# wangjunchi/LLMSeg

Measured on AMD Instinct MI355X. Metric: images/sec (1024x1024, 64-tok prompt) model_forward fwd+bwd, higher is better.
Workload: dtype bf16; 1 GPU; BASELINE.json configs[2]: synthetic 1024x1024 + random-init LLaVA-7B(Llama-7B+CLIP-L/14)/SAM-ViT-H, batch_size=2 per GPU, fwd+bwd train step (CE + align + IoP losses, LoRA r=8 dropout 0.05 on q/v + trainable embed/lm_head/text_fcs/lisa_*, frozen towers, fp32 gradient arena, AdamW step every 10 micro-steps inside the timed region, micro-step replayed from a hipGraph), 256 candidate masks, 64-token ; global_batch=2, parallelism=dp1, graph=True, valid=True

## Files before the change

llmseg_amd/csrc/backward.hip:

```cpp
#include <algorithm>
#include <cstdlib>
#include "common.h"
#include "llmseg_hip.h"

namespace {

inline unsigned grid_for(long total) {
  long g = (total + 255) / 256;
  return (unsigned)(g < 1 ? 1 : (g > 8192 ? 8192 : g));
}

__global__ __launch_bounds__(256) void colsum_kernel(const bf16_t* __restrict__ x, float* __restrict__ out, float* __restrict__ part, long M, long N, long ld) {
  __shared__ float red[4][64];
  const int c = threadIdx.x & 63, rl = threadIdx.x >> 6;
  const long col = (long)blockIdx.x * 64 + c;
  const long rows_per = (M + gridDim.y - 1) / gridDim.y;
  const long r0 = (long)blockIdx.y * rows_per, r1 = min(M, r0 + rows_per);
  float s = 0.f;
  if (col < N)
    for (long r = r0 + rl; r < r1; r += 4) s += bf2f(x[r * ld + col]);
  red[rl][c] = s;
  __syncthreads();
  if (rl == 0 && col < N) {
    const float v = (red[0][c] + red[1][c]) + (red[2][c] + red[3][c]);
// ... 505 lines not shown
}

extern "C" int llmseg_ce_bwd(const void* logits, const int64_t* labels, const float* coef, void* dlogits, int32_t N, int32_t T, int64_t V, int64_t ldl,
                             void* stream) {
  LL_CHECK(logits && labels && coef && dlogits && N > 0 && T > 1 && V > 0 && ldl >= V, "ce_bwd: bad arguments");
  LL_LAUNCH_KERNEL(ce_bwd_kernel, dim3((unsigned)(N * T)), dim3(256), 0, (hipStream_t)stream, (const bf16_t*)logits, labels, coef, (bf16_t*)dlogits, T,
                     (long)V, (long)ldl);
  LL_LAUNCH_CHECK("ce_bwd");
  return LLMSEG_OK;
}

extern "C" int llmseg_scatter_add_rows(const void* src, const int64_t* idx, float* dst, int64_t n, int64_t cols, void* stream) {
  LL_CHECK(src && idx && dst && n > 0 && cols > 0, "scatter_add_rows: bad arguments");
  LL_CHECK(n < (1L << 31), "scatter_add_rows: too many source rows");
  LL_LAUNCH_KERNEL(scatter_add_rows_kernel, dim3((unsigned)n), dim3(256), 0, (hipStream_t)stream, (const bf16_t*)src, idx, dst, (long)n, (long)cols);
  LL_LAUNCH_CHECK("scatter_add_rows");
  return LLMSEG_OK;
}

extern "C" int llmseg_sumsq(const void* x, int64_t n, int is_f32, float* out, void* workspace, int64_t workspace_bytes, void* stream) {
  LL_CHECK(x && out && n > 0, "sumsq: bad arguments");
  LL_CHECK(workspace && workspace_bytes >= 4, "sumsq: workspace (>= 4 bytes, 8 KiB for every partial) is required");
  long g = std::min<long>(2048, (n + 2047) / 2048);
  g = std::max<long>(1, std::min<long>(g, workspace_bytes / 4));
  LL_LAUNCH_KERNEL(sumsq_kernel, dim3((unsigned)g), dim3(256), 0, (hipStream_t)stream, x, (long)n, is_f32, (float*)workspace);
  LL_LAUNCH_KERNEL(fold_column_kernel, dim3(1), dim3(256), 0, (hipStream_t)stream, (const float*)workspace, (long)g, out, 1.f);
  LL_LAUNCH_CHECK("sumsq");
  return LLMSEG_OK;
}

extern "C" int llmseg_adamw(void* p, float* master, const void* grad, int grad_f32, float* m, float* v, int64_t n, float lr, float beta1, float beta2,
                            float eps, float weight_decay, int64_t step, const float* grad_scale, void* stream) {
  LL_CHECK(p && master && grad && m && v && n > 0 && step > 0, "adamw: bad arguments");
  const float bc1 = 1.f - powf(beta1, (float)step), bc2 = 1.f - powf(beta2, (float)step);
  LL_LAUNCH_KERNEL(adamw_kernel, dim3(grid_for(n)), dim3(256), 0, (hipStream_t)stream, (bf16_t*)p, master, grad, grad_f32, m, v, (long)n, lr, beta1, beta2,
                     eps, weight_decay, bc1, bc2, grad_scale);
  LL_LAUNCH_CHECK("adamw");
  return LLMSEG_OK;
}

namespace {
constexpr int LR = 8;

struct DropP { const unsigned long* rng; uint32_t stream, thr; float scale; uint32_t seg; };

__device__ __forceinline__ unsigned long drop_index(const DropP& dp, unsigned long m, unsigned long width, unsigned long k, uint32_t& off_add) {
  off_add = 0;
  if (dp.seg) {
    off_add = (uint32_t)(m / dp.seg);
    m -= (unsigned long)off_add * dp.seg;
  }
  return (m * width + k) >> 3;
}

template <int RW>
__global__ __launch_bounds__(256) void lora_down_kernel(const bf16_t* __restrict__ x0, const bf16_t* __restrict__ x1, long ldx, const bf16_t* __restrict__ w0,
                                                       const bf16_t* __restrict__ w1, bf16_t* __restrict__ y, long ldy, long M, int K, int w_kr, float alpha,
                                                       int zero_cols, int nb, DropP dp) {
  const int lane = threadIdx.x & 63;
  const long m0 = ((long)blockIdx.x * 4 + (threadIdx.x >> 6)) * RW;
  if (m0 >= M) return;
  float acc[2][RW][LR];
#pragma unroll
  for (int b = 0; b < 2; ++b)
#pragma unroll
    for (int i = 0; i < RW; ++i)
#pragma unroll
      for (int r = 0; r < LR; ++r) acc[b][i][r] = 0.f;
  const bool same = x0 == x1;
#pragma unroll 2
  for (int k = lane * 8; k < K; k += 64 * 8) {
#pragma unroll
    for (int b = 0; b < 2; ++b) {
      if (b >= nb) break;
      const bf16_t* xb = b == 0 ? x0 : x1;
      const bf16_t* wb = b == 0 ? w0 : w1;
      float xv[RW][8], wv[8];
#pragma unroll
      for (int i = 0; i < RW; ++i) {
        const long m = min(m0 + i, M - 1);
        unpack8(*reinterpret_cast<const uint4*>(xb + m * ldx + k), xv[i]);
        if (dp.thr) {
          uint32_t oa;
          const unsigned long di = drop_index(dp, (unsigned long)m, (unsigned long)K, (unsigned long)k, oa);
          dropout8(xv[i], di, dp.stream + b, dp.rng, dp.thr, dp.scale, oa);
        }
      }
      (void)same;
      if (w_kr) {
#pragma unroll
        for (int j = 0; j < 8; ++j) {
          unpack8(*reinterpret_cast<const uint4*>(wb + (long)(k + j) * LR), wv);
#pragma unroll
          for (int i = 0; i < RW; ++i)
#pragma unroll
            for (int r = 0; r < LR; ++r) acc[b][i][r] += xv[i][j] * wv[r];
        }
      } else {
#pragma unroll
        for (int r = 0; r < LR; ++r) {
          unpack8(*reinterpret_cast<const uint4*>(wb + (long)r * K + k), wv);
#pragma unroll
          for (int i = 0; i < RW; ++i)
#pragma unroll
            for (int j = 0; j < 8; ++j) acc[b][i][r] += xv[i][j] * wv[j];
        }
      }
    }
  }
#pragma unroll
  for (int i = 0; i < RW; ++i) {
#pragma unroll
    for (int b = 0; b < 2; ++b)
#pragma unroll
      for (int r = 0; r < LR; ++r) acc[b][i][r] = wave_sum(acc[b][i][r]) * alpha;
    if (m0 + i < M) {
      bf16_t* yr = y + (m0 + i) * ldy;
      if (lane == 0) *reinterpret_cast<uint4*>(yr) = pack8(acc[0][i]);
      else if (lane == 1 && nb > 1) *reinterpret_cast<uint4*>(yr + 8) = pack8(acc[1][i]);
      else if (lane >= nb && (lane - nb) * 8 < zero_cols) *reinterpret_cast<uint4*>(yr + lane * 8) = make_uint4(0, 0, 0, 0);
    }
  }
}

__global__ __launch_bounds__(256) void lora_down_mfma_kernel(const bf16_t* __restrict__ x0, const bf16_t* __restrict__ x1, long ldx, const bf16_t* __restrict__ w0,
                                                            const bf16_t* __restrict__ w1, bf16_t* __restrict__ y, long ldy, long M, int K, float alpha,
                                                            int zero_cols, int nb, DropP dp, float* __restrict__ part) {
  __shared__ float red[4][2][8][16];
  __shared__ float fin[16][16];
  const int lane = threadIdx.x & 63, wave = threadIdx.x >> 6;
  const int r = lane & 15, kc = lane >> 4;
  const long m0 = (long)blockIdx.x * 16;
  const long m = min(m0 + r, M - 1);
  const int kq = K / (4 * (int)gridDim.y);
  const int kbeg = ((int)blockIdx.y * 4 + wave) * kq;
  const bool same = x0 == x1;
  f32x4_t acc0 = {0.f, 0.f, 0.f, 0.f}, acc1 = {0.f, 0.f, 0.f, 0.f};
  auto masked = [&](uint4 v, unsigned long idx, uint32_t stream, uint32_t off_add) {
    const unsigned long seed = dp.rng[0], off = dp.rng[1] + off_add;
    const Philox8 ph = philox4x32_10((uint32_t)idx, (uint32_t)(idx >> 32), stream, (uint32_t)off, (uint32_t)seed, (uint32_t)(seed >> 32));
    uint32_t* u = reinterpret_cast<uint32_t*>(&v);
#pragma unroll
    for (int j = 0; j < 4; ++j) {
      const uint32_t lo = (ph.w[j] & 0xffffu) >= dp.thr ? 0x0000ffffu : 0u, hi = (ph.w[j] >> 16) >= dp.thr ? 0xffff0000u : 0u;
      u[j] &= lo | hi;
    }
    return v;
  };
#pragma unroll 4
  for (int k = kbeg + kc * 8; k < kbeg + kq; k += 32) {
    uint4 xa = *reinterpret_cast<const uint4*>(x0 + m * ldx + k);
    uint4 xb = (nb > 1 && !same) ? *reinterpret_cast<const uint4*>(x1 + m * ldx + k) : xa;
    const uint4 wa = r < LR ? *reinterpret_cast<const uint4*>(w0 + (long)r * K + k) : make_uint4(0, 0, 0, 0);
    const uint4 wb = (nb > 1 && r < LR) ? *reinterpret_cast<const uint4*>(w1 + (long)r * K + k) : make_uint4(0, 0, 0, 0);
    if (dp.thr) {
      uint32_t oa;
      const unsigned long idx = drop_index(dp, (unsigned long)m, (unsigned long)K, (unsigned long)k, oa);
      xa = masked(xa, idx, dp.stream, oa);
      if (nb > 1) xb = masked(xb, idx, dp.stream + 1, oa);
    }
    acc0 = __builtin_amdgcn_mfma_f32_16x16x32_bf16(__builtin_bit_cast(bf16x8_t, wa), __builtin_bit_cast(bf16x8_t, xa), acc0, 0, 0, 0);
    if (nb > 1) acc1 = __builtin_amdgcn_mfma_f32_16x16x32_bf16(__builtin_bit_cast(bf16x8_t, wb), __builtin_bit_cast(bf16x8_t, xb), acc1, 0, 0, 0);
  }
  if (kc < 2) {
#pragma unroll
    for (int e = 0; e < 4; ++e) { red[wave][0][4 * kc + e][r] = acc0[e]; red[wave][1][4 * kc + e][r] = acc1[e]; }
  }
  __syncthreads();
  {
    const int b = threadIdx.x >> 7, rank = (threadIdx.x >> 4) & 7, mm = threadIdx.x & 15;
    const float sum = (red[0][b][rank][mm] + red[1][b][rank][mm]) + (red[2][b][rank][mm] + red[3][b][rank][mm]);
    if (part) {
      if (m0 + mm < M) part[((long)blockIdx.y * M + m0 + mm) * 16 + b * 8 + rank] = sum;
    } else fin[mm][b * 8 + rank] = sum * alpha * (dp.thr ? dp.scale : 1.f);
  }
  if (part) return;
  __syncthreads();
  const int nch = nb + zero_cols / 8;
  for (int t = threadIdx.x; t < 16 * nch; t += blockDim.x) {
    const int mm = t / nch, ch = t - mm * nch;
    if (m0 + mm >= M) continue;
    uint4 o = make_uint4(0, 0, 0, 0);
    if (ch < nb) o = pack8(&fin[mm][ch * 8]);
    *reinterpret_cast<uint4*>(y + (m0 + mm) * ldy + ch * 8) = o;
  }
}

__device__ __forceinline__ void lora_down_finish_body(const float* __restrict__ part, int S, bf16_t* __restrict__ y, long ldy, long M, float scale,
                                                      int zero_cols, int nb, long bid, long nblocks) {
  const int nch = nb + zero_cols / 8;
  const long total = M * nch;
  for (long t = bid * blockDim.x + threadIdx.x; t < total; t += nblocks * blockDim.x) {
    const long mm = t / nch;
    const int ch = (int)(t - mm * nch);
    uint4 o = make_uint4(0, 0, 0, 0);
    if (ch < nb) {
      float v[8];
#pragma unroll
      for (int e = 0; e < 8; ++e) v[e] = 0.f;
      for (int s2 = 0; s2 < S; ++s2) {
        const float* pp = part + ((long)s2 * M + mm) * 16 + ch * 8;
#pragma unroll
        for (int e = 0; e < 8; ++e) v[e] += pp[e];
      }
#pragma unroll
      for (int e = 0; e < 8; ++e) v[e] *= scale;
      o = pack8(v);
    }
    *reinterpret_cast<uint4*>(y + mm * ldy + ch * 8) = o;
  }
}
__global__ __launch_bounds__(256) void lora_down_finish_kernel(const float* __restrict__ part, int S, bf16_t* __restrict__ y, long ldy, long M, float scale,
                                                              int zero_cols, int nb) {
  lora_down_finish_body(part, S, y, ldy, M, scale, zero_cols, nb, blockIdx.x, gridDim.x);
}

struct OuterP { const bf16_t* a[4]; const bf16_t* b[4]; float* out[4]; long lda[4], ldb[4]; int out_rn[4]; float alpha[4]; uint32_t drop[4]; };
__global__ __launch_bounds__(256) void lora_outer_kernel(OuterP q, long M, long N, DropP dp, float* __restrict__ part) {
  __shared__ float red[4][8][8 * LR];
  const int z = blockIdx.z;
  const bf16_t* __restrict__ a = q.a[z];
  const bf16_t* __restrict__ b = q.b[z];
  float* __restrict__ out = q.out[z];
  const long lda = q.lda[z], ldb = q.ldb[z];
  const int out_rn = q.out_rn[z];
  const float alpha = q.alpha[z];
  if (q.drop[z] == 0) dp.thr = 0;
  const uint32_t dstream = q.drop[z] - 1;
  const int lane = threadIdx.x & 63, wave = threadIdx.x >> 6;
  const int cl = lane & 7, rl = lane >> 3;
  const long n = ((long)blockIdx.x * 8 + cl) * 8;
  const long per = (M + gridDim.y * 4 - 1) / (gridDim.y * 4);
  const long m0 = ((long)blockIdx.y * 4 + wave) * per, m1 = min(M, m0 + per);
  const bool on = n < N;
  float acc[8][LR];
#pragma unroll
  for (int j = 0; j < 8; ++j)
#pragma unroll
    for (int r = 0; r < LR; ++r) acc[j][r] = 0.f;
  if (on) {
    long m = m0 + rl;
    for (; m + 16 < m1; m += 24) {
      uint4 av[3], bv[3];
#pragma unroll
      for (int u = 0; u < 3; ++u) {
        av[u] = *reinterpret_cast<const uint4*>(a + (m + 8 * u) * lda + n);
        bv[u] = *reinterpret_cast<const uint4*>(b + (m + 8 * u) * ldb);
      }
#pragma unroll
      for (int u = 0; u < 3; ++u) {
        float x[8], y[8];
        unpack8(av[u], x); unpack8(bv[u], y);
        if (dp.thr) {
          uint32_t oa;
          const unsigned long di = drop_index(dp, (unsigned long)(m + 8 * u), (unsigned long)N, (unsigned long)n, oa);
          dropout8(x, di, dstream, dp.rng, dp.thr, dp.scale, oa);
        }
#pragma unroll
        for (int j = 0; j < 8; ++j)
#pragma unroll
          for (int r = 0; r < LR; ++r) acc[j][r] = fmaf(x[j], y[r], acc[j][r]);
      }
    }
    for (; m < m1; m += 8) {
      float x[8], y[8];
      unpack8(*reinterpret_cast<const uint4*>(a + m * lda + n), x);
      unpack8(*reinterpret_cast<const uint4*>(b + m * ldb), y);
      if (dp.thr) {
        uint32_t oa;
        const unsigned long di = drop_index(dp, (unsigned long)m, (unsigned long)N, (unsigned long)n, oa);
        dropout8(x, di, dstream, dp.rng, dp.thr, dp.scale, oa);
      }
#pragma unroll
      for (int j = 0; j < 8; ++j)
#pragma unroll
        for (int r = 0; r < LR; ++r) acc[j][r] = fmaf(x[j], y[r], acc[j][r]);
    }
  }
#pragma unroll
  for (int j = 0; j < 8; ++j)
#pragma unroll
    for (int r = 0; r < LR; ++r) {
      float v = acc[j][r];
      v += __shfl_xor(v, 8, 64); v += __shfl_xor(v, 16, 64); v += __shfl_xor(v, 32, 64);
      acc[j][r] = v * alpha;
    }
  if (rl == 0) {
#pragma unroll
    for (int j = 0; j < 8; ++j)
#pragma unroll
      for (int r = 0; r < LR; ++r) red[wave][cl][j * LR + r] = acc[j][r];
  }
  __syncthreads();
  float* __restrict__ dstp = part ? part + ((long)blockIdx.y * gridDim.z + z) * N * LR : out;
  for (int idx = threadIdx.x; idx < 8 * 8 * LR; idx += blockDim.x) {
    const int c = idx / (8 * LR), jr = idx % (8 * LR), j = jr / LR, r = jr % LR;
    const long nn = ((long)blockIdx.x * 8 + c) * 8 + j;
    if (nn < N) {
      const float v = (red[0][c][jr] + red[1][c][jr]) + (red[2][c][jr] + red[3][c][jr]);
      const long cell = out_rn ? (long)r * N + nn : nn * LR + r;
      if (part) dstp[cell] = v;
      else dstp[cell] += v;
    }
  }
}

__global__ __launch_bounds__(256) void lora_apply_kernel(bf16_t* __restrict__ y, long ldy, const bf16_t* __restrict__ xa, long ldxa,
                                                        const bf16_t* __restrict__ w0, const bf16_t* __restrict__ w1, long M, long N, int w_rn,
                                                        float alpha, int nb, DropP dp) {
  const long nch = N >> 3, total = M * nch;
  for (long i = (long)blockIdx.x * blockDim.x + threadIdx.x; i < total; i += (long)gridDim.x * blockDim.x) {
    const long m = i / nch, c = i % nch;
    float yv[8], wv[8];
    unpack8(*reinterpret_cast<const uint4*>(y + m * ldy + c * 8), yv);
    for (int b = 0; b < nb; ++b) {
      const bf16_t* w = b == 0 ? w0 : w1;
      float xv[8], dv[8];
      unpack8(*reinterpret_cast<const uint4*>(xa + m * ldxa + 8 * b), xv);
      if (w_rn) {
#pragma unroll
        for (int j = 0; j < 8; ++j) dv[j] = 0.f;
#pragma unroll
        for (int r = 0; r < LR; ++r) {
          unpack8(*reinterpret_cast<const uint4*>(w + (long)r * N + c * 8), wv);
#pragma unroll
          for (int j = 0; j < 8; ++j) dv[j] += xv[r] * wv[j];
        }
      } else {
#pragma unroll
        for (int j = 0; j < 8; ++j) {
          unpack8(*reinterpret_cast<const uint4*>(w + (c * 8 + j) * LR), wv);
          float s = 0.f;
#pragma unroll
          for (int r = 0; r < LR; ++r) s += xv[r] * wv[r];
          dv[j] = s;
        }
      }
      if (dp.thr) {
        uint32_t oa;
        const unsigned long di = drop_index(dp, (unsigned long)m, (unsigned long)N, (unsigned long)(c * 8), oa);
        dropout8(dv, di, dp.stream + b, dp.rng, dp.thr, dp.scale, oa);
      }
#pragma unroll
      for (int j = 0; j < 8; ++j) yv[j] += alpha * dv[j];
    }
    *reinterpret_cast<uint4*>(y + m * ldy + c * 8) = pack8(yv);
  }
}

template <int CPT, bool LORA>
__global__ __launch_bounds__(256) void reduce_lora_normbwd_kernel(const float* __restrict__ slab, int S, long slab_sz, const bf16_t* __restrict__ x,
                                                                 const bf16_t* __restrict__ w, bf16_t* __restrict__ dx, long rows, int cols, float eps, int rms,
                                                                 const bf16_t* __restrict__ dres, bf16_t* __restrict__ xa, long ldxa,
                                                                 const bf16_t* __restrict__ w0, const bf16_t* __restrict__ w1, float alpha, int nb, DropP dp,
                                                                 const float* __restrict__ lp, int lS, float lscale, int lzero) {
  __shared__ float red[16];
  __shared__ float tl[16];
  const long row = blockIdx.x;
  const int nch = cols >> 3;
  const long N = cols;
  if (LORA && lp != nullptr) {
    if (threadIdx.x < 16) {
      float v = 0.f;
      if ((int)threadIdx.x < 8 * nb) {
        for (int s2 = 0; s2 < lS; ++s2) v += lp[((long)s2 * rows + row) * 16 + threadIdx.x];
        v *= lscale;
      }
      const bf16_t vb = f2bf(v);
      tl[threadIdx.x] = bf2f(vb);
      xa[row * ldxa + threadIdx.x] = vb;
    } else if ((int)threadIdx.x < 16 + lzero) xa[row * ldxa + threadIdx.x] = 0;
    __syncthreads();
  }
  uint4 xc[CPT], gc[CPT], wc[CPT];
#pragma unroll
  for (int i = 0; i < CPT; ++i) {
    const int c = threadIdx.x + 256 * i;
    xc[i] = gc[i] = wc[i] = make_uint4(0, 0, 0, 0);
    if (c < nch) {
      xc[i] = *reinterpret_cast<const uint4*>(x + row * cols + c * 8);
      wc[i] = *reinterpret_cast<const uint4*>(w + c * 8);
      const float* sp = slab + row * N + c * 8;
      float4 a0 = *reinterpret_cast<const float4*>(sp), a1 = *reinterpret_cast<const float4*>(sp + 4);
      for (int s2 = 1; s2 < S; ++s2) {
        const float4 b0 = *reinterpret_cast<const float4*>(sp + s2 * slab_sz), b1 = *reinterpret_cast<const float4*>(sp + s2 * slab_sz + 4);
        a0.x += b0.x; a0.y += b0.y; a0.z += b0.z; a0.w += b0.w;
        a1.x += b1.x; a1.y += b1.y; a1.z += b1.z; a1.w += b1.w;
      }
      const float v[8] = {a0.x, a0.y, a0.z, a0.w, a1.x, a1.y, a1.z, a1.w};
      gc[i] = pack8(v);
      if (LORA) {
        float yv[8], wv[8];
        unpack8(gc[i], yv);
        for (int b = 0; b < nb; ++b) {
          const bf16_t* wl = b == 0 ? w0 : w1;
          float xv[8], dv[8];
          if (lp != nullptr) {
#pragma unroll
            for (int r = 0; r < 8; ++r) xv[r] = tl[8 * b + r];
          } else unpack8(*reinterpret_cast<const uint4*>(xa + row * ldxa + 8 * b), xv);
#pragma unroll
          for (int j = 0; j < 8; ++j) dv[j] = 0.f;
#pragma unroll
          for (int r = 0; r < LR; ++r) {
            unpack8(*reinterpret_cast<const uint4*>(wl + (long)r * N + c * 8), wv);
#pragma unroll
            for (int j = 0; j < 8; ++j) dv[j] += xv[r] * wv[j];
          }
          if (dp.thr) {
            uint32_t oa;
            const unsigned long di = drop_index(dp, (unsigned long)row, (unsigned long)N, (unsigned long)(c * 8), oa);
            dropout8(dv, di, dp.stream + b, dp.rng, dp.thr, dp.scale, oa);
          }
#pragma unroll
          for (int j = 0; j < 8; ++j) yv[j] += alpha * dv[j];
        }
        gc[i] = pack8(yv);
      }
    }
  }
  normbwd_row<CPT>(xc, gc, wc, red, dx, row, cols, eps, rms, dres);
}

__device__ __forceinline__ void lora_pack_body(const bf16_t* __restrict__ aq, const bf16_t* __restrict__ bq, const bf16_t* __restrict__ av,
                                               const bf16_t* __restrict__ bv, bf16_t* __restrict__ w2b, bf16_t* __restrict__ w2a, bf16_t* __restrict__ bt,
                                               long H, float s, long bid, long nblocks) {
  const long total = 4 * H * 8 + (bt ? 2 * H : 0);
  for (long i = bid * blockDim.x + threadIdx.x; i < total; i += nblocks * blockDim.x) {
    if (i >= 4 * H * 8) {
      const long j = i - 4 * H * 8;
      const int row16 = (int)(j / (H >> 3));
      const long h0 = (j - (long)row16 * (H >> 3)) * 8;
      const bf16_t* src = row16 < 8 ? bq : bv;
      uint32_t o[4];
#pragma unroll
      for (int e = 0; e < 4; ++e) o[e] = (uint32_t)src[(h0 + 2 * e) * LR + (row16 & 7)] | ((uint32_t)src[(h0 + 2 * e + 1) * LR + (row16 & 7)] << 16);
      *reinterpret_cast<uint4*>(bt + (long)row16 * H + h0) = make_uint4(o[0], o[1], o[2], o[3]);
      continue;
    }
    const long row = i >> 3;
    const int ch = (int)(i & 7);
    float v[8] = {0.f, 0.f, 0.f, 0.f, 0.f, 0.f, 0.f, 0.f};
    if (row < 3 * H) {
      if (w2b == nullptr) continue;
      if (row < H && ch == 0) { unpack8(*reinterpret_cast<const uint4*>(bq + row * LR), v); }
      else if (row >= 2 * H && ch == 1) { unpack8(*reinterpret_cast<const uint4*>(bv + (row - 2 * H) * LR), v); }
#pragma unroll
      for (int j = 0; j < 8; ++j) v[j] *= s;
      *reinterpret_cast<uint4*>(w2b + row * 64 + ch * 8) = pack8(v);
    } else {
      if (w2a == nullptr) continue;
      const long h = row - 3 * H;
      if (ch < 2) {
        const bf16_t* src = ch == 0 ? aq : av;
#pragma unroll
        for (int r = 0; r < LR; ++r) v[r] = bf2f(src[(long)r * H + h]);
      }
      *reinterpret_cast<uint4*>(w2a + h * 64 + ch * 8) = pack8(v);
    }
  }
}
__global__ __launch_bounds__(256) void lora_pack_kernel(const bf16_t* __restrict__ aq, const bf16_t* __restrict__ bq, const bf16_t* __restrict__ av,
                                                       const bf16_t* __restrict__ bv, bf16_t* __restrict__ w2b, bf16_t* __restrict__ w2a, bf16_t* __restrict__ bt,
                                                       long H, float s) {
  lora_pack_body(aq, bq, av, bv, w2b, w2a, bt, H, s, blockIdx.x, gridDim.x);
}
__global__ __launch_bounds__(256) void lora_finish_pack_kernel(const float* __restrict__ part, int S, bf16_t* __restrict__ y, long ldy, long M, float scale, int zero_cols,
                                                              int nb, int gf, const bf16_t* __restrict__ aq, const bf16_t* __restrict__ bq,
                                                              const bf16_t* __restrict__ av, const bf16_t* __restrict__ bv, bf16_t* __restrict__ w2b,
                                                              bf16_t* __restrict__ w2a, bf16_t* __restrict__ bt, long H, float s) {
  if ((int)blockIdx.x < gf) lora_down_finish_body(part, S, y, ldy, M, scale, zero_cols, nb, blockIdx.x, gf);
  else lora_pack_body(aq, bq, av, bv, w2b, w2a, bt, H, s, (long)blockIdx.x - gf, (long)gridDim.x - gf);
}
__global__ __launch_bounds__(256) void transpose_pad_kernel(const bf16_t* __restrict__ in, bf16_t* __restrict__ out, long rows, long cols, long ld_in,
                                                           long ld_out, long rows_pad) {
  __shared__ bf16_t tile[64][66];
  const long r0 = (long)blockIdx.y * 64, c0 = (long)blockIdx.x * 64;
#pragma unroll
  for (int i = 0; i < 2; ++i) {
    const int idx = threadIdx.x + i * 256;
    const int r = idx >> 3, ch = idx & 7;
    uint4 v = make_uint4(0, 0, 0, 0);
    if (r0 + r < rows && c0 + ch * 8 < cols) v = *reinterpret_cast<const uint4*>(in + (r0 + r) * ld_in + c0 + ch * 8);
    uint32_t* dst = reinterpret_cast<uint32_t*>(&tile[r][ch * 8]);
    dst[0] = v.x; dst[1] = v.y; dst[2] = v.z; dst[3] = v.w;
  }
  __syncthreads();
#pragma unroll
  for (int i = 0; i < 2; ++i) {
    const int idx = threadIdx.x + i * 256;
    const int c = idx >> 3, rh = idx & 7;
    if (c0 + c >= cols || r0 + rh * 8 >= rows_pad) continue;
    uint32_t w[4];
#pragma unroll
    for (int j = 0; j < 4; ++j) w[j] = (uint32_t)tile[rh * 8 + 2 * j][c] | ((uint32_t)tile[rh * 8 + 2 * j + 1][c] << 16);
    *reinterpret_cast<uint4*>(out + (c0 + c) * ld_out + r0 + rh * 8) = make_uint4(w[0], w[1], w[2], w[3]);
  }
}

}

static DropP make_drop(const llmseg_dropout* d) {
  DropP dp{nullptr, 0u, 0u, 1.f, 0u};
  if (d && d->rng_state && d->drop_thr > 0) {
    dp.rng = (const unsigned long*)d->rng_state; dp.stream = d->stream; dp.thr = d->drop_thr; dp.seg = d->seg_rows;
    dp.scale = 65536.f / (65536.f - (float)d->drop_thr);
  }
  return dp;
}

extern "C" __attribute__((visibility("hidden"))) int llmseg_reduce_lora_normbwd(const float* slab, int S, int64_t M, int64_t N, const void* x, const void* w, void* dx, float eps,
                                                                                int rms, const void* dres, void* la_t, int64_t la_ldt, const void* la_w0,
                                                                                const void* la_w1, float la_alpha, const llmseg_dropout* la_drop, const float* la_part,
                                                                                int la_S, float la_scale, int la_zero, void* stream) {
  LL_CHECK(slab && S >= 1 && M > 0 && N >= 2048 && N <= 8192 && (N & 7) == 0 && x && w && dx && AL16(x) && AL16(w) && AL16(dx) && AL16(dres) && AL16(slab),
           "reduce_lora_normbwd: bad arguments");
  LL_CHECK(!la_t || (la_w0 && AL16(la_t) && AL16(la_w0) && AL16(la_w1) && (la_ldt & 7) == 0), "reduce_lora_normbwd: bad LoRA operands");
  LL_CHECK(!la_part || (la_t && la_S >= 1 && la_zero >= 0 && la_zero <= 240 && la_ldt >= 16 + la_zero), "reduce_lora_normbwd: bad LoRA partials");
  const DropP dp = make_drop(la_drop);
  const int cpt = (int)(((N >> 3) + 255) / 256), nb = la_w1 ? 2 : 1;
#define LL_RLN(C, L)                                                                                                                                     \
  LL_LAUNCH_KERNEL((reduce_lora_normbwd_kernel<C, L>), dim3((unsigned)M), dim3(256), 0, (hipStream_t)stream, slab, S, (long)(M * N), (const bf16_t*)x,    \
                   (const bf16_t*)w, (bf16_t*)dx, (long)M, (int)N, eps, rms, (const bf16_t*)dres, (bf16_t*)la_t, (long)la_ldt, (const bf16_t*)la_w0, \
                   (const bf16_t*)la_w1, la_alpha, nb, dp, la_part, la_S, la_scale, la_zero)
  if (la_t) { if (cpt <= 1) LL_RLN(1, true); else if (cpt <= 2) LL_RLN(2, true); else LL_RLN(4, true); }
  else { if (cpt <= 1) LL_RLN(1, false); else if (cpt <= 2) LL_RLN(2, false); else LL_RLN(4, false); }
#undef LL_RLN
  LL_LAUNCH_CHECK("reduce_lora_normbwd");
  return LLMSEG_OK;
}
#define LL_DROP_OK(d) (!(d) || (d)->drop_thr < 65536u)

extern "C" int llmseg_lora_down(const void* x0, const void* x1, int64_t ldx, const void* w0, const void* w1, void* y, int64_t ldy, int64_t M, int64_t K,
                                int32_t w_kr, float alpha, int32_t zero_cols, const llmseg_dropout* drop, void* stream) {
  return llmseg_lora_down_ws(x0, x1, ldx, w0, w1, y, ldy, M, K, w_kr, alpha, zero_cols, drop, nullptr, 0, stream);
}

struct PartsReq { bool active, done; int S; float scale; };
static thread_local PartsReq g_parts_req = {false, false, 0, 0.f};
struct PackReq { const bf16_t *aq, *bq, *av, *bv; bf16_t *w2b, *w2a, *bt; long H; float s; bool active, done; };
static thread_local PackReq g_pack_req = {nullptr, nullptr, nullptr, nullptr, nullptr, nullptr, nullptr, 0, 0.f, false, false};

extern "C" int llmseg_lora_down_ws(const void* x0, const void* x1, int64_t ldx, const void* w0, const void* w1, void* y, int64_t ldy, int64_t M, int64_t K,
                                   int32_t w_kr, float alpha, int32_t zero_cols, const llmseg_dropout* drop, void* scratch, int64_t scratch_bytes, void* stream) {
  const int nb = (x1 && w1) ? 2 : 1;
  LL_CHECK(x0 && w0 && y && (!x1) == (!w1) && M > 0 && K > 0 && (K & 7) == 0 && (ldx & 7) == 0 && (ldy & 7) == 0 && ldy >= 8 * nb + zero_cols &&
               zero_cols >= 0 && (zero_cols & 7) == 0 && zero_cols <= 480 && AL16(x0) && AL16(x1) && AL16(w0) && AL16(w1) && AL16(y) && LL_DROP_OK(drop),
           "lora_down: bad arguments");
  const DropP dp = make_drop(drop);
  const bf16_t *X0 = (const bf16_t*)x0, *X1 = (const bf16_t*)(x1 ? x1 : x0), *W0 = (const bf16_t*)w0, *W1 = (const bf16_t*)(w1 ? w1 : w0);
  static const int force = getenv("LLMSEG_LORA_DOWN") ? atoi(getenv("LLMSEG_LORA_DOWN")) : 0;
  if (!w_kr && (K & 127) == 0 && force != 1) {
    if (force == 2) scratch = nullptr;
    const long tiles = (M + 15) / 16;
    int S = 1;
    while (tiles * S < 256 && (K % (4 * 32 * S * 2)) == 0 && scratch && (int64_t)S * 2 * M * 16 * 4 <= scratch_bytes && S < 32) S *= 2;
    float* part = S > 1 ? (float*)scratch : nullptr;
    LL_LAUNCH_KERNEL(lora_down_mfma_kernel, dim3((unsigned)tiles, (unsigned)S), dim3(256), 0, (hipStream_t)stream, X0, X1, (long)ldx, W0, W1, (bf16_t*)y, (long)ldy,
                       (long)M, (int)K, alpha, zero_cols, nb, dp, part);
    if (S > 1 && g_parts_req.active) {
      g_parts_req.done = true; g_parts_req.S = S; g_parts_req.scale = alpha * (dp.thr ? dp.scale : 1.f);
    } else if (S > 1 && g_pack_req.active) {
      const PackReq& q = g_pack_req;
      const unsigned gf = grid_for(M * (nb + zero_cols / 8)), gp = grid_for(4 * q.H * 8 + 2 * q.H);
      LL_LAUNCH_KERNEL(lora_finish_pack_kernel, dim3(gf + gp), dim3(256), 0, (hipStream_t)stream, (const float*)part, S, (bf16_t*)y, (long)ldy, (long)M,
                         alpha * (dp.thr ? dp.scale : 1.f), zero_cols, nb, (int)gf, q.aq, q.bq, q.av, q.bv, q.w2b, q.w2a, q.bt, q.H, q.s);
      g_pack_req.done = true;
    } else if (S > 1)
      LL_LAUNCH_KERNEL(lora_down_finish_kernel, dim3(grid_for(M * (nb + zero_cols / 8))), dim3(256), 0, (hipStream_t)stream, (const float*)part, S, (bf16_t*)y,
                         (long)ldy, (long)M, alpha * (dp.thr ? dp.scale : 1.f), zero_cols, nb);
  } else if (M <= 2048)
    LL_LAUNCH_KERNEL(lora_down_kernel<1>, dim3((unsigned)((M + 3) / 4)), dim3(256), 0, (hipStream_t)stream, X0, X1, (long)ldx, W0, W1, (bf16_t*)y, (long)ldy, (long)M,
                       (int)K, w_kr, alpha, zero_cols, nb, dp);
  else
    LL_LAUNCH_KERNEL(lora_down_kernel<4>, dim3((unsigned)((M + 15) / 16)), dim3(256), 0, (hipStream_t)stream, X0, X1, (long)ldx, W0, W1, (bf16_t*)y, (long)ldy, (long)M,
                       (int)K, w_kr, alpha, zero_cols, nb, dp);
  LL_LAUNCH_CHECK("lora_down");
  return LLMSEG_OK;
}

static int lora_outer_launch(const OuterP& q, int nz, int64_t M, int64_t N, const DropP& dp, void* workspace, int64_t workspace_bytes, hipStream_t stream) {
  const long colwg = (N + 63) / 64;
  long gy = max(max((long)1, 256 / (colwg * nz)), min((long)32, M / 512));
  gy = min(gy, workspace ? (long)(workspace_bytes / (nz * N * LR * 4)) : 0L);
  float* part = gy > 1 ? (float*)workspace : nullptr;
  if (gy < 1) gy = 1;
  LL_LAUNCH_KERNEL(lora_outer_kernel, dim3((unsigned)colwg, (unsigned)gy, (unsigned)nz), dim3(256), 0, stream, q, (long)M, (long)N, dp, part);
  if (part)
    LL_LAUNCH_KERNEL(fold_slices_kernel, dim3(fold_grid(nz * N * LR)), dim3(256), 0, stream, (const float*)part, (int)gy, (long)(nz * N * LR),
                     (long)(nz * N * LR), (long)(N * LR), FoldOut{{q.out[0], q.out[1], q.out[2], q.out[3]}});
  LL_LAUNCH_CHECK("lora_outer");
  return LLMSEG_OK;
}

extern "C" int llmseg_lora_outer(const void* a0, const void* a1, int64_t lda, const void* b0, const void* b1, int64_t ldb, float* out0, float* out1, int64_t M,
                                 int64_t N, int32_t out_rn, float alpha, const llmseg_dropout* drop, void* workspace, int64_t workspace_bytes, void* stream) {
  const int nz = (a1 && b1 && out1) ? 2 : 1;
  LL_CHECK(a0 && b0 && out0 && ((!a1) == (!b1)) && ((!a1) == (!out1)) && M > 0 && N > 0 && (N & 7) == 0 && (lda & 7) == 0 && (ldb & 7) == 0 && AL16(a0) &&
               AL16(a1) && AL16(b0) && AL16(b1) && LL_DROP_OK(drop), "lora_outer: bad arguments (N, lda, ldb multiples of 8)");
  OuterP q{};
  const DropP dp = make_drop(drop);
  for (int z = 0; z < nz; ++z) {
    q.a[z] = (const bf16_t*)(z ? a1 : a0); q.b[z] = (const bf16_t*)(z ? b1 : b0); q.out[z] = z ? out1 : out0;
    q.lda[z] = lda; q.ldb[z] = ldb; q.out_rn[z] = out_rn; q.alpha[z] = alpha; q.drop[z] = dp.thr ? dp.stream + z + 1 : 0;
  }
  return lora_outer_launch(q, nz, M, N, dp, workspace, workspace_bytes, (hipStream_t)stream);
}

extern "C" int llmseg_lora_wgrads(const void* dq, const void* dv, int64_t ldd, const void* x, int64_t ldx, const void* xa, int64_t ldxa, const void* t,
                                  int64_t ldt, float* gbq, float* gbv, float* gaq, float* gav, int64_t M, int64_t H, float s, const llmseg_dropout* drop,
                                  void* workspace, int64_t workspace_bytes, void* stream) {
  LL_CHECK(dq && dv && x && xa && t && gbq && gbv && gaq && gav && M > 0 && H > 0 && (H & 7) == 0 && (ldd & 7) == 0 && (ldx & 7) == 0 && (ldxa & 7) == 0 &&
               (ldt & 7) == 0 && ldxa >= 16 && ldt >= 16 && AL16(dq) && AL16(dv) && AL16(x) && AL16(xa) && AL16(t) && LL_DROP_OK(drop),
           "lora_wgrads: bad arguments");
  const DropP dp = make_drop(drop);
  OuterP q{};
  q.a[0] = (const bf16_t*)dq; q.b[0] = (const bf16_t*)xa;     q.out[0] = gbq; q.lda[0] = ldd; q.ldb[0] = ldxa; q.out_rn[0] = 0; q.alpha[0] = s;   q.drop[0] = 0;
  q.a[1] = (const bf16_t*)dv; q.b[1] = (const bf16_t*)xa + 8; q.out[1] = gbv; q.lda[1] = ldd; q.ldb[1] = ldxa; q.out_rn[1] = 0; q.alpha[1] = s;   q.drop[1] = 0;
  q.a[2] = (const bf16_t*)x;  q.b[2] = (const bf16_t*)t;      q.out[2] = gaq; q.lda[2] = ldx; q.ldb[2] = ldt;  q.out_rn[2] = 1; q.alpha[2] = 1.f; q.drop[2] = dp.thr ? dp.stream + 1 : 0;
  q.a[3] = (const bf16_t*)x;  q.b[3] = (const bf16_t*)t + 8;  q.out[3] = gav; q.lda[3] = ldx; q.ldb[3] = ldt;  q.out_rn[3] = 1; q.alpha[3] = 1.f; q.drop[3] = dp.thr ? dp.stream + 2 : 0;
  return lora_outer_launch(q, 4, M, H, dp, workspace, workspace_bytes, (hipStream_t)stream);
}

extern "C" int llmseg_lora_apply(void* y, int64_t ldy, const void* xa, int64_t ldxa, const void* w0, const void* w1, int64_t M, int64_t N, int32_t w_rn,
                                 float alpha, const llmseg_dropout* drop, void* stream) {
  LL_CHECK(y && xa && w0 && M > 0 && N > 0 && (N & 7) == 0 && (ldy & 7) == 0 && (ldxa & 7) == 0 && ldxa >= (w1 ? 16 : 8) && AL16(y) && AL16(xa) && AL16(w0) &&
               AL16(w1) && LL_DROP_OK(drop), "lora_apply: bad arguments");
  LL_CHECK(!(drop && drop->drop_thr) || ldy == N, "lora_apply: the dropout mask indexes y as a dense [M][N] matrix");
  LL_LAUNCH_KERNEL(lora_apply_kernel, dim3(grid_for(M * (N >> 3))), dim3(256), 0, (hipStream_t)stream, (bf16_t*)y, (long)ldy, (const bf16_t*)xa,
                     (long)ldxa, (const bf16_t*)w0, (const bf16_t*)w1, (long)M, (long)N, w_rn, alpha, w1 ? 2 : 1, make_drop(drop));
  LL_LAUNCH_CHECK("lora_apply");
  return LLMSEG_OK;
}

extern "C" int llmseg_lora_pack(const void* aq, const void* bq, const void* av, const void* bv, void* w2b, void* w2a, void* bt, int64_t H, float s, void* stream) {
  LL_CHECK(aq && bq && av && bv && (w2b || w2a || bt) && H > 0 && (H & 7) == 0 && AL16(aq) && AL16(bq) && AL16(av) && AL16(bv) && AL16(w2b) && AL16(w2a) && AL16(bt),
           "lora_pack: bad arguments");
  LL_LAUNCH_KERNEL(lora_pack_kernel, dim3(grid_for(4 * H * 8 + 2 * H)), dim3(256), 0, (hipStream_t)stream, (const bf16_t*)aq, (const bf16_t*)bq, (const bf16_t*)av,
                     (const bf16_t*)bv, (bf16_t*)w2b, (bf16_t*)w2a, (bf16_t*)bt, (long)H, s);
  LL_LAUNCH_CHECK("lora_pack");
  return LLMSEG_OK;
}

extern "C" int llmseg_lora_down_parts(const void* x0, const void* x1, int64_t ldx, const void* w0, const void* w1, void* y, int64_t ldy, int64_t M, int64_t K,
                                      int32_t w_kr, float alpha, int32_t zero_cols, const llmseg_dropout* drop, void* scratch, int64_t scratch_bytes, int32_t* S_out,
                                      float* scale_out, void* stream) {
  LL_CHECK(S_out && scale_out, "lora_down_parts: S_out / scale_out");
  static const bool off = getenv("LLMSEG_NO_LORA_PARTS") != nullptr;
  g_parts_req = PartsReq{!off, false, 0, 0.f};
  const int rc = llmseg_lora_down_ws(x0, x1, ldx, w0, w1, y, ldy, M, K, w_kr, alpha, zero_cols, drop, scratch, scratch_bytes, stream);
  *S_out = g_parts_req.done ? g_parts_req.S : 0;
  *scale_out = g_parts_req.scale;
  g_parts_req.active = false;
  return rc;
}
extern "C" __attribute__((visibility("hidden"))) int llmseg_lora_down_finish(const float* part, int S, void* y, int64_t ldy, int64_t M, float scale, int zero_cols, int nb, void* stream) {
  LL_LAUNCH_KERNEL(lora_down_finish_kernel, dim3(grid_for(M * (nb + zero_cols / 8))), dim3(256), 0, (hipStream_t)stream, part, S, (bf16_t*)y, (long)ldy, (long)M, scale,
                     zero_cols, nb);
  LL_LAUNCH_CHECK("lora_down_finish");
  return LLMSEG_OK;
}

extern "C" int llmseg_lora_down_pack(const void* x0, const void* x1, int64_t ldx, const void* w0, const void* w1, void* y, int64_t ldy, int64_t M, int64_t K,
                                     int32_t w_kr, float alpha, int32_t zero_cols, const llmseg_dropout* drop, void* scratch, int64_t scratch_bytes, const void* aq,
                                     const void* bq, const void* av, const void* bv, void* w2b, void* w2a, void* bt, int64_t H, float s, void* stream) {
  LL_CHECK(aq && bq && av && bv && (w2b || w2a || bt) && H > 0 && (H & 7) == 0 && AL16(aq) && AL16(bq) && AL16(av) && AL16(bv) && AL16(w2b) && AL16(w2a) && AL16(bt),
           "lora_down_pack: bad pack arguments");
  static const bool off = getenv("LLMSEG_NO_FINISH_PACK") != nullptr;
  g_pack_req = PackReq{(const bf16_t*)aq, (const bf16_t*)bq, (const bf16_t*)av, (const bf16_t*)bv, (bf16_t*)w2b, (bf16_t*)w2a, (bf16_t*)bt, (long)H, s, !off, false};
  const int rc = llmseg_lora_down_ws(x0, x1, ldx, w0, w1, y, ldy, M, K, w_kr, alpha, zero_cols, drop, scratch, scratch_bytes, stream);
  const bool done = g_pack_req.done;
  g_pack_req.active = false;
  if (rc != LLMSEG_OK || done) return rc;
  return llmseg_lora_pack(aq, bq, av, bv, w2b, w2a, bt, H, s, stream);
}

extern "C" int llmseg_transpose_pad(const void* in, void* out, int64_t rows, int64_t cols, int64_t ld_in, int64_t ld_out, int64_t rows_pad, void* stream) {
  LL_CHECK(in && out && rows > 0 && cols > 0 && rows_pad >= rows && ld_out >= rows_pad && ld_in >= cols, "transpose_pad: bad arguments");
  LL_CHECK((cols & 7) == 0 && (ld_in & 7) == 0 && (ld_out & 7) == 0 && (rows_pad & 7) == 0 && AL16(in) && AL16(out),
           "transpose_pad: cols, rows_pad and leading dimensions must be multiples of 8, pointers 16-byte aligned");
  LL_LAUNCH_KERNEL(transpose_pad_kernel, dim3((unsigned)((cols + 63) / 64), (unsigned)((rows_pad + 63) / 64)), dim3(256), 0, (hipStream_t)stream,
                     (const bf16_t*)in, (bf16_t*)out, (long)rows, (long)cols, (long)ld_in, (long)ld_out, (long)rows_pad);
  LL_LAUNCH_CHECK("transpose_pad");
  return LLMSEG_OK;
}

namespace {
constexpr int LB_TI = 32, LB_TK = 64, LB_CC = 256, LB_LD = LB_CC + 8;

struct LinBwd {
  const bf16_t *dy, *y, *x, *w;
  bf16_t* dx;
  float *dw, *db;
  int M, N, K, act, accumulate;
  int w_it, w_kt, x_kt;
  int vec_n, vec_k;
};

__device__ __forceinline__ uint4 lb_load8(const bf16_t* __restrict__ p, int r, int c, int rows, int cols, bool vec) {
  if (r >= rows || c >= cols) return make_uint4(0, 0, 0, 0);
  const bf16_t* q = p + (long)r * cols + c;
  if (vec) return *reinterpret_cast<const uint4*>(q);
  uint32_t h[8];
#pragma unroll
  for (int j = 0; j < 8; ++j) h[j] = c + j < cols ? (uint32_t)q[j] : 0u;
  return make_uint4(h[0] | (h[1] << 16), h[2] | (h[3] << 16), h[4] | (h[5] << 16), h[6] | (h[7] << 16));
}

__device__ __forceinline__ uint4 lb_act8(const uint4& g, const uint4& yv, int act) {
  if (act == LLMSEG_ACT_NONE) return g;
  float gf[8], yf[8];
  uint32_t o[8];
  unpack8(g, gf); unpack8(yv, yf);
#pragma unroll
  for (int e = 0; e < 8; ++e) o[e] = f2bf(act == LLMSEG_ACT_RELU ? (yf[e] > 0.f ? gf[e] : 0.f) : gf[e] * yf[e] * (1.f - yf[e]));
  return make_uint4(o[0] | (o[1] << 16), o[2] | (o[3] << 16), o[4] | (o[5] << 16), o[6] | (o[7] << 16));
}

__device__ __forceinline__ uint32_t lb_elem(const uint4& v, int j) {
  const uint32_t wd = (j >> 1) == 0 ? v.x : (j >> 1) == 1 ? v.y : (j >> 1) == 2 ? v.z : v.w;
  return (j & 1) ? (wd >> 16) : (wd & 0xffffu);
}

__device__ __forceinline__ void lb_store_t(bf16_t* T, int col0, int c, const uint4& lo, const uint4& hi) {
#pragma unroll
  for (int j = 0; j < 8; ++j) *reinterpret_cast<uint32_t*>(T + (col0 + j) * LB_LD + c) = lb_elem(lo, j) | (lb_elem(hi, j) << 16);
}

__global__ __launch_bounds__(256) void linear_bwd_kernel(const LinBwd p) {
  __shared__ __attribute__((aligned(16))) bf16_t lds[(LB_TI + LB_TK) * LB_LD];
  bf16_t* AT = lds;
  bf16_t* BT = lds + LB_TI * LB_LD;
  const int t = threadIdx.x, lane = t & 63, wave = t >> 6;
  const int nW = p.w_it * p.w_kt;
  const bool roleW = (int)blockIdx.x < nW;
  const int bi = roleW ? (int)blockIdx.x : (int)blockIdx.x - nW;
  const int nkt = roleW ? p.w_kt : p.x_kt;
  const int i0 = (bi / nkt) * LB_TI, k0 = (bi % nkt) * LB_TK;
  const int C = roleW ? p.M : p.N;
  const bf16_t* __restrict__ B = roleW ? p.x : p.w;
  const bool vn = p.vec_n != 0, vk = p.vec_k != 0, has_act = p.act != LLMSEG_ACT_NONE;
  const bool want_db = roleW && (bi % nkt) == 0 && p.db != nullptr;

  uint4 ra[4], ry[4], rb[8];
  auto load_chunk = [&](int c0) {
#pragma unroll
    for (int q = 0; q < 4; ++q) {
      int r, c;
      if (roleW) { const int pr = t + 256 * (q >> 1); r = c0 + 2 * (pr >> 2) + (q & 1); c = i0 + 8 * (pr & 3); }
      else { const int v = t + 256 * q; r = i0 + (v >> 5); c = c0 + 8 * (v & 31); }
      ra[q] = lb_load8(p.dy, r, c, p.M, p.N, vn);
      if (has_act) ry[q] = lb_load8(p.y, r, c, p.M, p.N, vn);
    }
#pragma unroll
    for (int q = 0; q < 8; ++q) {
      const int pr = t + 256 * (q >> 1);
      rb[q] = lb_load8(B, c0 + 2 * (pr >> 3) + (q & 1), k0 + 8 * (pr & 7), C, p.K, vk);
    }
  };
  auto store_chunk = [&]() {
    if (has_act) {
#pragma unroll
      for (int q = 0; q < 4; ++q) ra[q] = lb_act8(ra[q], ry[q], p.act);
    }
    if (roleW) {
#pragma unroll
      for (int q = 0; q < 2; ++q) { const int pr = t + 256 * q; lb_store_t(AT, 8 * (pr & 3), 2 * (pr >> 2), ra[2 * q], ra[2 * q + 1]); }
    } else {
#pragma unroll
      for (int q = 0; q < 4; ++q) { const int v = t + 256 * q; *reinterpret_cast<uint4*>(AT + (v >> 5) * LB_LD + 8 * (v & 31)) = ra[q]; }
    }
#pragma unroll
    for (int q = 0; q < 4; ++q) { const int pr = t + 256 * q; lb_store_t(BT, 8 * (pr & 7), 2 * (pr >> 3), rb[2 * q], rb[2 * q + 1]); }
  };

  f32x4_t acc[2][4];
#pragma unroll
  for (int ib = 0; ib < 2; ++ib)
#pragma unroll
    for (int kb = 0; kb < 4; ++kb) acc[ib][kb] = f32x4_t{0.f, 0.f, 0.f, 0.f};
  float dbacc = 0.f;

  const int nch = (C + LB_CC - 1) / LB_CC;
  load_chunk(0);
  for (int ch = 0; ch < nch; ++ch) {
    if (ch) __syncthreads();
    store_chunk();
    __syncthreads();
    if (ch + 1 < nch) load_chunk((ch + 1) * LB_CC);
    if (want_db) {
      const bf16_t* row = AT + (t >> 3) * LB_LD + 32 * (t & 7);
#pragma unroll
      for (int v = 0; v < 4; ++v) {
        float f[8];
        unpack8(*reinterpret_cast<const uint4*>(row + 8 * v), f);
#pragma unroll
        for (int e = 0; e < 8; ++e) dbacc += f[e];
      }
    }
#pragma unroll
    for (int ks = 0; ks < 2; ++ks) {
      const int cw = wave * 64 + ks * 32;
      if (ch * LB_CC + cw >= C) break;
      const int cb = cw + 8 * (lane >> 4);
      bf16x8_t af[2], bf[4];
#pragma unroll
      for (int ib = 0; ib < 2; ++ib) af[ib] = *reinterpret_cast<const bf16x8_t*>(AT + (16 * ib + (lane & 15)) * LB_LD + cb);
#pragma unroll
      for (int kb = 0; kb < 4; ++kb) bf[kb] = *reinterpret_cast<const bf16x8_t*>(BT + (16 * kb + (lane & 15)) * LB_LD + cb);
#pragma unroll
      for (int ib = 0; ib < 2; ++ib)
#pragma unroll
        for (int kb = 0; kb < 4; ++kb) acc[ib][kb] = __builtin_amdgcn_mfma_f32_16x16x32_bf16(af[ib], bf[kb], acc[ib][kb], 0, 0, 0);
    }
  }

  if (want_db) {
    dbacc += __shfl_xor(dbacc, 4, 64);
    dbacc += __shfl_xor(dbacc, 2, 64);
    dbacc += __shfl_xor(dbacc, 1, 64);
    const int n = i0 + (t >> 3);
    if ((t & 7) == 0 && n < p.N) p.db[n] = p.accumulate ? p.db[n] + dbacc : dbacc;
  }
  if (roleW && !p.dw) return;

  float* fold = reinterpret_cast<float*>(lds);
  __syncthreads();
#pragma unroll
  for (int ib = 0; ib < 2; ++ib)
#pragma unroll
    for (int kb = 0; kb < 4; ++kb)
#pragma unroll
      for (int e = 0; e < 4; ++e) fold[(wave * LB_TI + 16 * ib + 4 * (lane >> 4) + e) * LB_TK + 16 * kb + (lane & 15)] = acc[ib][kb][e];
  __syncthreads();
#pragma unroll
  for (int q = 0; q < 8; ++q) {
    const int idx = t + 256 * q, i = idx >> 6, k = idx & 63;
    float s = fold[idx];
    s += fold[LB_TI * LB_TK + idx];
    s += fold[2 * LB_TI * LB_TK + idx];
    s += fold[3 * LB_TI * LB_TK + idx];
    const int gi = i0 + i, gk = k0 + k;
    if (gk >= p.K) continue;
    if (roleW) {
      if (gi < p.N) { float* o = p.dw + (long)gi * p.K + gk; *o = p.accumulate ? *o + s : s; }
    } else if (gi < p.M) {
      p.dx[(long)gi * p.K + gk] = f2bf(s);
    }
  }
}
}

extern "C" int llmseg_linear_bwd(const void* dy, const void* y, int act, const void* x, const void* w, void* dx, float* dw, float* db, int64_t M, int64_t N, int64_t K,
                                 int accumulate, void* stream) {
  LL_CHECK(dy && x && w && M > 0 && N > 0 && K > 0 && (dx || dw || db), "linear_bwd: bad arguments");
  LL_CHECK(act == LLMSEG_ACT_NONE || ((act == LLMSEG_ACT_RELU || act == LLMSEG_ACT_SIGMOID) && y), "linear_bwd: only relu/sigmoid are differentiated, from the output y");
  if (M > 2048 || N * K > (1L << 22)) return LLMSEG_NOT_TAKEN;
  LinBwd p;
  p.dy = (const bf16_t*)dy; p.y = (const bf16_t*)y; p.x = (const bf16_t*)x; p.w = (const bf16_t*)w;
  p.dx = (bf16_t*)dx; p.dw = dw; p.db = db;
  p.M = (int)M; p.N = (int)N; p.K = (int)K; p.act = act; p.accumulate = accumulate ? 1 : 0;
  p.w_it = (dw || db) ? (int)((N + LB_TI - 1) / LB_TI) : 0;
  p.w_kt = dw ? (int)((K + LB_TK - 1) / LB_TK) : 1;
  p.x_kt = (int)((K + LB_TK - 1) / LB_TK);
  p.vec_n = (N & 7) == 0 && AL16(dy) && (act == LLMSEG_ACT_NONE || AL16(y));
  p.vec_k = (K & 7) == 0 && AL16(x) && AL16(w);
  const long grid = (long)p.w_it * p.w_kt + (dx ? (long)((M + LB_TI - 1) / LB_TI) * p.x_kt : 0L);
  LL_LAUNCH_KERNEL(linear_bwd_kernel, dim3((unsigned)grid), dim3(256), 0, (hipStream_t)stream, p);
  LL_LAUNCH_CHECK("linear_bwd");
  return LLMSEG_OK;
}
```

Measured before the change: 52.94 images/s.

## Add wide 512-thread LoRA outer-product gradient kernel with prefetch and shuffle reduction

```diff
diff --git a/llmseg_amd/csrc/backward.hip b/llmseg_amd/csrc/backward.hip
--- a/llmseg_amd/csrc/backward.hip
+++ b/llmseg_amd/csrc/backward.hip
@@ -831,6 +831,167 @@
       if (part) dstp[cell] = v;
       else dstp[cell] += v;
     }
+  }
+}
+
+__device__ __forceinline__ void dropout8_m64(float* f, unsigned long idx, uint32_t stream, const unsigned long* rng, uint32_t thr, float scale, uint32_t off_add) {
+  const unsigned long seed = rng[0], off = rng[1] + off_add;
+  uint32_t c0 = (uint32_t)idx, c1 = (uint32_t)(idx >> 32), c2 = stream, c3 = (uint32_t)off, k0 = (uint32_t)seed, k1 = (uint32_t)(seed >> 32);
+#pragma unroll
+  for (int r = 0; r < 10; ++r) {
+    const unsigned long p0 = (unsigned long)0xD2511F53u * c0, p1 = (unsigned long)0xCD9E8D57u * c2;
+    c0 = (uint32_t)(p1 >> 32) ^ c1 ^ k0; c1 = (uint32_t)p1; c2 = (uint32_t)(p0 >> 32) ^ c3 ^ k1; c3 = (uint32_t)p0;
+    k0 += 0x9E3779B9u; k1 += 0xBB67AE85u;
+  }
+  const uint32_t w[4] = {c0, c1, c2, c3};
+#pragma unroll
+  for (int j = 0; j < 8; ++j) {
+    const uint32_t field = (w[j >> 1] >> (16 * (j & 1))) & 0xffffu;
+    f[j] = field >= thr ? f[j] * scale : 0.f;
+  }
+}
+
+struct OuterZ { int p0[4], p1[4]; };
+constexpr int OU_U = 3;
+struct OuterCell { int p, z, c, k; long cell; bool own; };
+__device__ __forceinline__ OuterCell outer_cell(const OuterP& q, int t, int pz0, int pz1, int np, unsigned bx, long N) {
+  OuterCell o;
+  const int tp = __builtin_amdgcn_readfirstlane(t >> 8), idx = t & 255;
+  o.p = tp < np ? tp : 0;
+  o.z = o.p ? pz1 : pz0;
+  const int rn = q.out_rn[o.z];
+  const int r = rn ? idx >> 5 : idx & 7, j = rn ? idx & 7 : (idx >> 3) & 7;
+  o.c = rn ? (idx >> 3) & 3 : idx >> 6;
+  o.k = j * LR + r;
+  const long nn = ((long)bx * 4 + o.c) * 8 + j;
+  o.own = tp < np && nn < N;
+  o.cell = rn ? (long)r * N + nn : nn * LR + r;
+  return o;
+}
+template <bool PAIR>
+__global__ __launch_bounds__(512) void lora_outer_wide_kernel(OuterP q, OuterZ zm, int nz, long M, long N, DropP dp, float* __restrict__ part) {
+  constexpr int NP = PAIR ? 2 : 1;
+  __shared__ float red[NP][8][4][8 * LR];
+  const int pz0 = zm.p0[blockIdx.z], pz1 = PAIR ? zm.p1[blockIdx.z] : -1;
+  const int np = pz1 >= 0 ? 2 : 1;
+  const bf16_t* __restrict__ a = q.a[pz0];
+  const long lda = q.lda[pz0];
+  const bf16_t* b[NP];
+  long ldb[NP];
+  uint32_t thr[NP], dstream[NP];
+#pragma unroll
+  for (int p = 0; p < NP; ++p) {
+    const int z = (p == 1 && np == 2) ? pz1 : pz0;
+    b[p] = q.b[z]; ldb[p] = q.ldb[z];
+    thr[p] = q.drop[z] ? dp.thr : 0; dstream[p] = q.drop[z] - 1;
+  }
+  const bool masked = thr[0] != 0 || (PAIR && thr[NP - 1] != 0);
+  const int lane = threadIdx.x & 63, wave = threadIdx.x >> 6;
+  const int cl = lane & 3, rl = lane >> 2;
+  const unsigned bx = (gridDim.x & 15) == 0 ? ((blockIdx.x & ~15u) | ((blockIdx.x & 7u) << 1) | ((blockIdx.x >> 3) & 1u)) : blockIdx.x;
+  const long n = ((long)bx * 4 + cl) * 8;
+  float old = 0.f;
+  {
+    const OuterCell o = outer_cell(q, (int)threadIdx.x, pz0, pz1, np, bx, N);
+    if (o.own && !part) old = q.out[o.z][o.cell];
+  }
+  const long sl = 4 * ((M + gridDim.y * 4 - 1) / (gridDim.y * 4));
+  const long s0 = (long)blockIdx.y * sl, s1 = min(M, s0 + sl);
+  float acc[NP][8][LR];
+#pragma unroll
+  for (int p = 0; p < NP; ++p)
+#pragma unroll
+    for (int j = 0; j < 8; ++j)
+#pragma unroll
+      for (int r = 0; r < LR; ++r) acc[p][j][r] = 0.f;
+  const long mb = s0 + wave * 16 + rl;
+  if (n < N && mb < s1) {
+    uint32_t sg = 0;
+    unsigned long rs = (unsigned long)mb;
+    if (masked && dp.seg) { sg = (uint32_t)(rs / dp.seg); rs -= (unsigned long)sg * dp.seg; }
+    unsigned long de = rs * (unsigned long)N + (unsigned long)n;
+    const unsigned long de_step = 128ul * (unsigned long)N, de_seg = (unsigned long)dp.seg * (unsigned long)N;
+    const bf16_t* pa = a + mb * lda + n;
+    const long sa = 128 * lda;
+    const bf16_t* pb[NP];
+    long sb[NP];
+#pragma unroll
+    for (int p = 0; p < NP; ++p) { pb[p] = b[p] + mb * ldb[p]; sb[p] = 128 * ldb[p]; }
+    uint4 av[OU_U], bv[NP][OU_U];
+#pragma unroll
+    for (int u = 0; u < OU_U; ++u) {
+      av[u] = make_uint4(0, 0, 0, 0);
+#pragma unroll
+      for (int p = 0; p < NP; ++p) bv[p][u] = make_uint4(0, 0, 0, 0);
+      if (mb + 128 * u < s1) {
+        av[u] = *reinterpret_cast<const uint4*>(pa + u * sa);
+#pragma unroll
+        for (int p = 0; p < NP; ++p)
+          if (p < np) bv[p][u] = *reinterpret_cast<const uint4*>(pb[p] + u * sb[p]);
+      }
+    }
+    for (long mt = mb; mt < s1; mt += 128 * OU_U) {
+#pragma unroll
+      for (int u = 0; u < OU_U; ++u) {
+        const long m = mt + 128 * u;
+        if (m < s1) {
+          float x0[8];
+          unpack8(av[u], x0);
+#pragma unroll
+          for (int p = 0; p < NP; ++p) {
+            if (p < np) {
+              float x[8], y[8];
+#pragma unroll
+              for (int j = 0; j < 8; ++j) x[j] = x0[j];
+              unpack8(bv[p][u], y);
+              if (thr[p]) dropout8_m64(x, de >> 3, dstream[p], dp.rng, thr[p], dp.scale, sg);
+#pragma unroll
+              for (int j = 0; j < 8; ++j)
+#pragma unroll
+                for (int r = 0; r < LR; ++r) acc[p][j][r] = fmaf(x[j], y[r], acc[p][j][r]);
+            }
+          }
+        }
+        rs += 128; de += de_step;
+        if (masked && dp.seg)
+          while (rs >= dp.seg) { rs -= dp.seg; de -= de_seg; ++sg; }
+        if (m + 128 * OU_U < s1) {
+          av[u] = *reinterpret_cast<const uint4*>(pa + (u + OU_U) * sa);
+#pragma unroll
+          for (int p = 0; p < NP; ++p)
+            if (p < np) bv[p][u] = *reinterpret_cast<const uint4*>(pb[p] + (u + OU_U) * sb[p]);
+        }
+      }
+      pa += OU_U * sa;
+#pragma unroll
+      for (int p = 0; p < NP; ++p) pb[p] += OU_U * sb[p];
+    }
+  }
+#pragma unroll
+  for (int p = 0; p < NP; ++p) {
+    if (p < np) {
+      float* v = &acc[p][0][0];
+#pragma unroll
+      for (int h = 32; h >= 4; h >>= 1) {
+        const bool hi = (lane & h) != 0;
+#pragma unroll
+        for (int i = 0; i < h; ++i) {
+          const float keep = hi ? v[i + h] : v[i], send = hi ? v[i] : v[i + h];
+          v[i] = keep + __shfl_xor(send, h, 64);
+        }
+      }
+      *reinterpret_cast<float4*>(&red[p][wave][cl][4 * rl]) = make_float4(v[0], v[1], v[2], v[3]);
+    }
+  }
+  __syncthreads();
+  int t = (int)threadIdx.x;
+  asm volatile("" : "+v"(t));
+  const OuterCell o = outer_cell(q, t, pz0, pz1, np, bx, N);
+  if (o.own) {
+    const float v = (((red[o.p][0][o.c][o.k] + red[o.p][1][o.c][o.k]) + (red[o.p][2][o.c][o.k] + red[o.p][3][o.c][o.k])) +
+                     ((red[o.p][4][o.c][o.k] + red[o.p][5][o.c][o.k]) + (red[o.p][6][o.c][o.k] + red[o.p][7][o.c][o.k]))) * q.alpha[o.z];
+    if (part) part[((long)blockIdx.y * nz + o.z) * N * LR + o.cell] = v;
+    else q.out[o.z][o.cell] = old + v;
   }
 }
 
@@ -1114,7 +1275,25 @@
   gy = min(gy, workspace ? (long)(workspace_bytes / (nz * N * LR * 4)) : 0L);
   float* part = gy > 1 ? (float*)workspace : nullptr;
   if (gy < 1) gy = 1;
-  LL_LAUNCH_KERNEL(lora_outer_kernel, dim3((unsigned)colwg, (unsigned)gy, (unsigned)nz), dim3(256), 0, stream, q, (long)M, (long)N, dp, part);
+  static const int form = getenv("LLMSEG_LORA_OUTER_V1") ? atoi(getenv("LLMSEG_LORA_OUTER_V1")) : 0;
+  if (form == 1) {
+    LL_LAUNCH_KERNEL(lora_outer_kernel, dim3((unsigned)colwg, (unsigned)gy, (unsigned)nz), dim3(256), 0, stream, q, (long)M, (long)N, dp, part);
+  } else {
+    OuterZ zm{};
+    int nzg = 0;
+    bool used[4] = {false, false, false, false}, pair = false;
+    for (int pass = 0; pass < 2; ++pass)
+      for (int z = 0; z < nz; ++z) {
+        if (used[z] || (pass == 0 && !q.drop[z])) continue;
+        used[z] = true; zm.p0[nzg] = z; zm.p1[nzg] = -1;
+        for (int w = z + 1; w < nz && form == 2; ++w)
+          if (!used[w] && q.a[w] == q.a[z] && q.lda[w] == q.lda[z]) { used[w] = true; zm.p1[nzg] = w; pair = true; break; }
+        ++nzg;
+      }
+    const dim3 grid((unsigned)((N + 31) / 32), (unsigned)gy, (unsigned)nzg);
+    if (pair) LL_LAUNCH_KERNEL(lora_outer_wide_kernel<true>, grid, dim3(512), 0, stream, q, zm, nz, (long)M, (long)N, dp, part);
+    else LL_LAUNCH_KERNEL(lora_outer_wide_kernel<false>, grid, dim3(512), 0, stream, q, zm, nz, (long)M, (long)N, dp, part);
+  }
   if (part)
     LL_LAUNCH_KERNEL(fold_slices_kernel, dim3(fold_grid(nz * N * LR)), dim3(256), 0, stream, (const float*)part, (int)gy, (long)(nz * N * LR),
                      (long)(nz * N * LR), (long)(N * LR), FoldOut{{q.out[0], q.out[1], q.out[2], q.out[3]}});
```

After: 53.24 images/s, median of 6. Within noise of the previous version (+0.6%).
